# balkce/beamform

Hardware: AMD Instinct MI355X
Metric: stft_frames_per_sec (higher is better)
Workload: dtype f64; 1 GPU; das 8-mic 1024-pt (hop 512), 65536-frame batch per GPU, 1 stream(s), planar input resident in HBM; frames_per_gpu=65536, frames_fed_per_gpu=65536, mics=8, fft=1024, hop=512, streams=1, layout=planar, gather=n/a, parallelism=independent batches x1, input=uniform noise in [-0.5, 0.5), settle_launches_before_warmup=416, forward_transforms_per_frame_pair=6

## Files before the change

beamform_amd/csrc/das_f64_w64.hip:

```cpp
#include <hip/hip_runtime.h>

#include <type_traits>

#include "launch_trace.hpp"
#include "pipeline_kernels.hpp"
#include "w64_f64_dev.hpp"

namespace bf {

namespace {

constexpr int kBlock = 512;
constexpr int kWaves = kBlock / 64;
constexpr int kHop = 512;
constexpr int kTwD = 2 * (1024 + 4 * kTw2RowW64Rot);
constexpr int oTw = 0;
constexpr int oPlane = kTwD;
constexpr int oGain = oPlane + kWaves * kPlaneD;
constexpr int oCross = oGain + 4 * 2048;
constexpr int oFlag = oCross + 512;
constexpr int kWinRow = 18;
constexpr int oWin = oFlag + 8;
constexpr int kLdsD = oWin + 64 * kWinRow;

// ... 180 lines not shown
        BF_STAGE();
        mul_tw<true, 1, 16>(Sr, Si, tw);
        BF_STAGE();
        load_tw1<1, 16>(tw, s_tw1, lane);
        BF_STAGE();
        fft16_core<double, +1, false>(Sr, Si);
        BF_STAGE();
        T1_inv(Sr, Si, row16, wcol);
        BF_STAGE();
        mul_tw<true, 1, 16>(Sr, Si, tw);
        fft16_core<double, +1, false>(Sr, Si);

        float o[16];
#pragma unroll
        for (int j = 0; j < 16; ++j) {
            const float f = (float)Sr[j];
            o[j] = (float)((double)f * wrow[j]);
        }
        const int pw = (w + kWaves - 1) & (kWaves - 1);
        if (t + 1 < T1) {
            float *area = (w < kWaves - 1) ? reinterpret_cast<float *>(plane) : s_cross + (it & 1) * kHop;
            if (w == kWaves - 1 && it >= 2)
                while (s_cons[w] < (int)(t - 2 * kWaves)) __builtin_amdgcn_s_sleep(1);
            asm volatile("" ::: "memory");
#pragma unroll
            for (int j = 0; j < 8; ++j) area[64 * j + lane] = o[j + 8];
            asm volatile("" ::: "memory");
            if (lane == 0) s_ready[w] = (int)t;
        }
        float *yo = ys + t * kHop;
        if (t == T0) {
            if (T0 == 0) {
                const float *ti = a.tail_in + (long)stream * kHop;
#pragma unroll
                for (int j = 0; j < 8; ++j) yo[(unsigned)(64 * j + lane)] = ti[(unsigned)(64 * j + lane)] + o[j];
            } else {
#pragma unroll
                for (int j = 0; j < 8; ++j) atomicAdd(yo + (unsigned)(64 * j + lane), o[j]);
            }
        } else {
            const float *parea = (pw < kWaves - 1) ? reinterpret_cast<const float *>(lds + oPlane + pw * kPlaneD) : s_cross + ((it + 1) & 1) * kHop;
            while (s_ready[pw] < (int)(t - 1)) __builtin_amdgcn_s_sleep(1);
            asm volatile("" ::: "memory");
            float prev[8];
#pragma unroll
            for (int j = 0; j < 8; ++j) prev[j] = parea[64 * j + lane];
            asm volatile("" ::: "memory");
            if (lane == 0) s_cons[pw] = (int)(t - 1);
#pragma unroll
            for (int j = 0; j < 8; ++j) yo[(unsigned)(64 * j + lane)] = prev[j] + o[j];
        }
        if (t == T1 - 1) {
            if (T1 < a.n_frames) {
                float *yn = ys + T1 * kHop;
#pragma unroll
                for (int j = 0; j < 8; ++j) atomicAdd(yn + (unsigned)(64 * j + lane), o[j + 8]);
            } else {
                float *to = a.tail_out + (long)stream * kHop;
#pragma unroll
                for (int j = 0; j < 8; ++j) to[(unsigned)(64 * j + lane)] = o[j + 8];
            }
        }
    }
}


#ifdef BF_PARK_PLAIN
#define BF_PARK_LD(p) (*(const volatile float *)(p))
#else
#define BF_PARK_LD(p) __builtin_nontemporal_load(p)
#endif
constexpr int kGRow = 65;
constexpr int kGMic = 8 * kGRow;
constexpr int kSlots = 64;
constexpr int kTwP = 2 * (960 + 4 * kTw2RowW64Rot);
constexpr int pTw = 0;
constexpr int pPlane = kTwP;
constexpr int pGain = pPlane + kWaves * kPlaneD;
constexpr int pFlag = pGain + 7 * kGMic * 2;
constexpr int kRingR = 32;
constexpr int kRingSlots = kRingR + kWaves;
constexpr int pRing = pFlag + (kSlots + 4) / 2;
constexpr int pWin = pRing + kRingR / 2;
constexpr int kLdsP = pWin + 64 * kWinRow;
static_assert(kLdsP * 8 <= 160 * 1024, "LDS");
static_assert((pGain & 1) == 0 && (pWin & 1) == 0, "16-byte alignment");


typedef volatile __attribute__((address_space(3))) int *lds_int_t;
typedef volatile __attribute__((address_space(3))) unsigned long long *lds_u64_t;
__device__ __forceinline__ int lds_fetch_add(lds_int_t p, int v, int lane) {
    int old = 0;
    if (lane == 0) old = __hip_atomic_fetch_add((__attribute__((address_space(3))) int *)p, v, __ATOMIC_RELAXED, __HIP_MEMORY_SCOPE_WORKGROUP);
    return __builtin_amdgcn_readfirstlane(old);
}
__device__ __forceinline__ unsigned long long lds_fetch_add64(lds_u64_t p, int lane) {
    unsigned long long old = 0;
    if (lane == 0) old = __hip_atomic_fetch_add((__attribute__((address_space(3))) unsigned long long *)p, 1ull, __ATOMIC_RELAXED, __HIP_MEMORY_SCOPE_WORKGROUP);
    const unsigned lo = (unsigned)__builtin_amdgcn_readfirstlane((int)(unsigned)old), hi = (unsigned)__builtin_amdgcn_readfirstlane((int)(unsigned)(old >> 32));
    return ((unsigned long long)hi << 32) | lo;
}
struct DasSched {
    const int4 *chunks;
    unsigned *counter;
    int n_chunks;
};
__device__ __forceinline__ unsigned long long pack_work(unsigned vbase, int chunk, int pairs, int next) {
    return ((unsigned long long)(vbase & 0xFFFFFFu) << 40) | ((unsigned long long)(unsigned)chunk << 20) | ((unsigned long long)(unsigned)pairs << 10) | (unsigned)next;
}
struct PairWork {
    int4 d;
    int pos;
    int len;
    unsigned u;
    bool have;
};
__device__ __forceinline__ int4 load_chunk(const int4 *chunks, int k) {
    const int4 d = chunks[k];
    return int4{__builtin_amdgcn_readfirstlane(d.x), __builtin_amdgcn_readfirstlane(d.y), __builtin_amdgcn_readfirstlane(d.z), k};
}
__device__ __forceinline__ PairWork draw_pair(lds_u64_t work, const DasSched &sc, int lane, const int4 held) {
    PairWork r;
    r.have = false;
    r.d = int4{0, 0, 0, 0};
    r.pos = r.len = 0;
    r.u = 0;
    for (;;) {
        const unsigned long long old = lds_fetch_add64(work, lane);
        const int pos = (int)(old & 1023u), len = (int)((old >> 10) & 1023u), k = (int)((old >> 20) & 0xFFFFFu);
        const unsigned vb = (unsigned)(old >> 40);
        if (k == kChunkEnd) return r;
        if (pos < len) {
            if (k == held.w) r.d = held;
            else r.d = load_chunk(sc.chunks, k);
            r.pos = pos; r.len = len; r.u = vb + (unsigned)pos; r.have = true;
            return r;
        }
        if (pos == len) {
            unsigned k2 = 0;
            if (lane == 0) k2 = __hip_atomic_fetch_add(sc.counter, 1u, __ATOMIC_RELAXED, __HIP_MEMORY_SCOPE_AGENT);
            k2 = (unsigned)__builtin_amdgcn_readfirstlane((int)k2);
            if (k2 >= (unsigned)sc.n_chunks) {
                if (lane == 0) *work = pack_work(vb + (unsigned)len, kChunkEnd, 0, 0);
                return r;
            }
            r.d = load_chunk(sc.chunks, (int)k2);
            r.len = (r.d.z + 1) >> 1;
            r.pos = 0; r.u = vb + (unsigned)len; r.have = true;
            if (lane == 0) *work = pack_work(r.u, (int)k2, r.len, 1);
            return r;
        }
        while ((int)((*work >> 20) & 0xFFFFFu) == k) __builtin_amdgcn_s_sleep(2);
    }
}
__device__ __forceinline__ int claim_boundary(lds_int_t st, unsigned b, int lane) {
    const int base = 4 * (int)(b / kSlots);
    while (st[b & (kSlots - 1)] < base) __builtin_amdgcn_s_sleep(1);
    return lds_fetch_add(st + (b & (kSlots - 1)), 1, lane) - base;
}
__device__ __forceinline__ void publish_boundary(lds_int_t st, unsigned b, int lane) { (void)lds_fetch_add(st + (b & (kSlots - 1)), 2, lane); }
__device__ __forceinline__ void skip_boundary(lds_int_t st, unsigned b, int lane) {
    const int base = 4 * (int)(b / kSlots);
    while (st[b & (kSlots - 1)] < base) __builtin_amdgcn_s_sleep(1);
    (void)lds_fetch_add(st + (b & (kSlots - 1)), 4, lane);
}
__device__ __forceinline__ void await_boundary(lds_int_t st, unsigned b) {
    while (st[b & (kSlots - 1)] - 4 * (int)(b / kSlots) < 3) __builtin_amdgcn_s_sleep(1);
}

#ifdef BF_W64_STATS
__device__ unsigned long long g_stats[256 * 8 * 5];
#define BF_STATS_DECL unsigned long long st_[5] = {0, 0, 0, 0, 0}; const unsigned long long st_t0_ = __builtin_amdgcn_s_memrealtime()
#define BF_STAT(i) (++st_[i])
#define BF_STAT_WAIT_BEGIN const unsigned long long st_w0_ = __builtin_amdgcn_s_memrealtime()
#define BF_STAT_WAIT_END st_[3] += __builtin_amdgcn_s_memrealtime() - st_w0_
#define BF_STATS_FLUSH do { st_[4] = __builtin_amdgcn_s_memrealtime() - st_t0_; if (lane == 0 && blockIdx.x < 256) for (int i_ = 0; i_ < 5; ++i_) g_stats[(blockIdx.x * 8 + w) * 5 + i_] = st_[i_]; } while (0)
#else
#define BF_STATS_DECL
#define BF_STAT(i) ((void)0)
#define BF_STAT_WAIT_BEGIN
#define BF_STAT_WAIT_END
#define BF_STATS_FLUSH
#endif
#ifdef BF_W64_STAMPS
__device__ unsigned long long g_stamps[256 * 8 * 64];
#define BF_STAMP(slot) do { if (lane == 0 && blockIdx.x < 256 && (slot) < 64) g_stamps[(blockIdx.x * 8 + w) * 64 + (slot)] = __builtin_amdgcn_s_memrealtime(); } while (0)
#else
#define BF_STAMP(slot) do { } while (0)
#endif

typedef float il_f4 __attribute__((ext_vector_type(4)));
template <int LG>
__device__ __forceinline__ void il_tile_through_plane(const il_f4 (&v)[4], float *tile, float *dst, int t, int lane) {
    constexpr int M = 1 << LG, R1 = LG == 3 ? 10 : M + 1, spt = 1024 >> LG;
    asm volatile("" : "+v"(lane)::"memory");
#pragma unroll
    for (int i = 0; i < 4; ++i) {
#pragma unroll
        for (int c = 0; c < 4; ++c) {
            const int e = 256 * i + 4 * lane + c;
            tile[(e >> LG) * R1 + (e & (M - 1))] = v[i][c];
        }
    }
    asm volatile("" ::: "memory");
    __builtin_amdgcn_wave_barrier();
#pragma unroll
    for (int j = 0; j < 4; ++j) {
        const int mic = lane & (M - 1), q4 = (lane >> LG) + (64 >> LG) * j;
        il_f4 o;
#pragma unroll
        for (int c = 0; c < 4; ++c) o[c] = tile[(4 * q4 + c) * R1 + mic];
        reinterpret_cast<il_f4 *>(dst + mic * kHop + t * spt)[q4] = o;
    }
    asm volatile("" ::: "memory");
    __builtin_amdgcn_wave_barrier();
}

template <int LAYOUT>
__device__ __forceinline__ void das_f64_pair_body(const DasF64Args &a, const DasSched &sc) {
    __shared__ __attribute__((aligned(16))) double lds[kLdsP];
    const cx<double> *s_tw1 = reinterpret_cast<const cx<double> *>(lds + pTw) - 64;
    const cx<double> *s_tw2 = reinterpret_cast<const cx<double> *>(lds + pTw) + 960;
    const cx<double> *s_gain = reinterpret_cast<const cx<double> *>(lds + pGain);
    lds_int_t s_state = (lds_int_t)(lds + pFlag);
    lds_u64_t s_work = (lds_u64_t)(lds + pFlag + kSlots / 2);
    lds_int_t s_ring = (lds_int_t)(lds + pRing);
    (void)s_ring;

    const int tid = threadIdx.x, lane = tid & 63;
    const int w = __builtin_amdgcn_readfirstlane(tid >> 6);
    const int M = a.n_mics;
    double *plane = lds + pPlane + w * kPlaneD;
    double *wcol = plane + w64_col_rot(lane);
    double *row16 = plane + (lane & 15) * kRS + 16 * (lane >> 4);
    const double *wrow = lds + pWin + lane * kWinRow;
    typedef double cxa __attribute__((ext_vector_type(2)));
    typedef const __attribute__((address_space(3))) cxa *lds_gain_t;
    unsigned gd0 = (unsigned)(size_t)(lds_gain_t)(s_gain + lane);
    asm volatile("" : "+v"(gd0));
    gd0 &= ~15u;
    const unsigned g_mirror = 2u * (unsigned)(size_t)(lds_gain_t)s_gain + 1024u;

    float n0[8], n1[8], n2[8];
#ifndef BF_PAIR_NT
#define BF_PAIR_NT 0
#endif
    auto request = [&](const float *h0, const float *h1, const float *h2) {
#pragma unroll
        for (int j = 0; j < 8; ++j) {
            n0[j] = (BF_PAIR_NT & 2) ? __builtin_nontemporal_load(h0 + (unsigned)(64 * j + lane)) : h0[(unsigned)(64 * j + lane)];
            n1[j] = (BF_PAIR_NT & 1) ? __builtin_nontemporal_load(h1 + (unsigned)(64 * j + lane)) : h1[(unsigned)(64 * j + lane)];
            n2[j] = (BF_PAIR_NT & 4) ? __builtin_nontemporal_load(h2 + (unsigned)(64 * j + lane)) : h2[(unsigned)(64 * j + lane)];
        }
    };
    auto request_pair_mic = [&](int stream, long tA, int m) {
        const float *h1 = a.x + (long)stream * a.stream_stride_x + (long)m * a.mic_stride + tA * kHop;
        const float *h0 = tA >= 1 ? h1 - kHop : a.hist + ((long)stream * M + m) * kHop;
        const float *h2 = tA + 1 < a.n_frames ? h1 + kHop : h1;
        request(h0, h1, h2);
    };
    float q0[8], q1[8], q2[8];
    const double inv_m = 1.0 / (double)M;
    float e0[8], e1[8], e2[8];
    const int NT = a.n_tr, XM = a.extra_mic;
    auto request_extra = [&](bool on, int stream, long tA) {
        if (!on) {
#pragma unroll
            for (int j = 0; j < 8; ++j) e0[j] = e1[j] = e2[j] = 0.f;
            return;
        }
        const float *h1 = a.x + (long)stream * a.stream_stride_x + (long)XM * a.mic_stride + tA * kHop;
        const float *h0 = tA >= 1 ? h1 - kHop : a.hist + ((long)stream * M + XM) * kHop;
        const float *h2 = tA + 1 < a.n_frames ? h1 + kHop : h1;
#pragma unroll
        for (int j = 0; j < 8; ++j) {
            e0[j] = h0[(unsigned)(64 * j + lane)];
            e1[j] = h1[(unsigned)(64 * j + lane)];
            e2[j] = h2[(unsigned)(64 * j + lane)];
        }
    };

    struct RingHops { const float *h, *a, *b; };
    typedef float f4 __attribute__((ext_vector_type(4)));
    const int lgM = 31 - __builtin_clz((unsigned)M);
    float *ringb = LAYOUT == 1 ? a.ring + (size_t)blockIdx.x * kRingSlots * M * kHop : nullptr;
    auto ring_slot = [&](unsigned j) { return ringb + (size_t)(j & (kRingR - 1)) * M * kHop; };
    auto il_load2 = [&](const float *src, int unit, f4 (&v)[2][4]) {
        const f4 *s4 = reinterpret_cast<const f4 *>(src);
#pragma unroll
        for (int tt = 0; tt < 2; ++tt) {
            const int t = 2 * unit + tt;
            if (2 * t < M) {
#pragma unroll
                for (int i = 0; i < 4; ++i) v[tt][i] = s4[t * 256 + i * 64 + lane];
            } else {
#pragma unroll
                for (int i = 0; i < 4; ++i) v[tt][i] = f4{0.f, 0.f, 0.f, 0.f};
            }
        }
    };
    auto il_store2 = [&](const f4 (&v)[2][4], float *dst, int unit) {
        float *tile = reinterpret_cast<float *>(plane);
#pragma unroll
        for (int tt = 0; tt < 2; ++tt) {
            const int t = 2 * unit + tt;
            if (2 * t < M) {
                if (lgM == 3) il_tile_through_plane<3>(v[tt], tile, dst, t, lane);
                else if (lgM == 2) il_tile_through_plane<2>(v[tt], tile, dst, t, lane);
                else il_tile_through_plane<1>(v[tt], tile, dst, t, lane);
            }
// ... 1 lines not shown
    };
    auto prepare_pair = [&](const PairWork &pw) {
        RingHops r;
        const unsigned u2 = 2u * pw.u;
        const int sA = (int)(u2 & (kRingR - 1)), gen4 = 4 * (int)(u2 / kRingR);
        float *dA = ring_slot(u2), *dB = ring_slot(u2 + 1), *dH = ringb + (size_t)(kRingR + w) * M * kHop;
        const long tA = pw.d.y + 2L * pw.pos;
        const float *xs = a.x + (long)pw.d.x * a.stream_stride_x;
        while (s_ring[sA] < gen4 || s_ring[sA + 1] < gen4) __builtin_amdgcn_s_sleep(1);
        f4 v0[2][4], v1[2][4];
        const bool two = tA + 1 < a.n_frames, first = pw.pos == 0, wide = M > 4;
        const float *srcA = xs + tA * (long)kHop * M, *srcB = srcA + (long)kHop * M;
        const float *srcH = tA >= 1 ? srcA - (long)kHop * M : a.hist + (long)pw.d.x * M * kHop;
        il_load2(srcA, 0, v0);
        if (wide) il_load2(srcA, 1, v1);
        il_store2(v0, dA, 0);
        if (two) il_load2(srcB, 0, v0);
        if (wide) il_store2(v1, dA, 1);
        if (two && wide) il_load2(srcB, 1, v1);
        if (two) il_store2(v0, dB, 0);
        if (first) il_load2(srcH, 0, v0);
        if (two && wide) il_store2(v1, dB, 1);
        if (first && wide) il_load2(srcH, 1, v1);
        if (first) il_store2(v0, dH, 0);
        if (first && wide) il_store2(v1, dH, 1);
        __builtin_amdgcn_fence(__ATOMIC_RELEASE, "workgroup");
        (void)lds_fetch_add(s_ring + sA, 2, lane);
        (void)lds_fetch_add(s_ring + sA + 1, 2, lane);
        r.a = dA;
        r.b = two ? dB : dA;
        r.h = dH;
        if (!first) {
            const unsigned jp = u2 - 1;
            const int sP = (int)(jp & (kRingR - 1)), genp = 4 * (int)(jp / kRingR);
            while (s_ring[sP] - genp < 2) __builtin_amdgcn_s_sleep(1);
            r.h = ring_slot(jp);
        }
        __builtin_amdgcn_fence(__ATOMIC_ACQUIRE, "workgroup");
        return r;
    };
    auto release_pair = [&](const PairWork &pw, bool has_t) {
        const unsigned u2 = 2u * pw.u;
        (void)lds_fetch_add(s_ring + (u2 & (kRingR - 1)), 2, lane);
        (void)lds_fetch_add(s_ring + ((u2 + 1) & (kRingR - 1)), has_t ? 1 : 2, lane);
        if (pw.pos > 0) (void)lds_fetch_add(s_ring + ((u2 - 1) & (kRingR - 1)), 1, lane);
    };
    auto request_ring_mic = [&](const RingHops &r, int m) { request(r.h + m * kHop, r.a + m * kHop, r.b + m * kHop); };
    auto request_ring_extra = [&](bool on, const RingHops &r) {
        if (!on) {
#pragma unroll
            for (int j = 0; j < 8; ++j) e0[j] = e1[j] = e2[j] = 0.f;
            return;
        }
#pragma unroll
        for (int j = 0; j < 8; ++j) {
            e0[j] = r.h[XM * kHop + (unsigned)(64 * j + lane)];
            e1[j] = r.a[XM * kHop + (unsigned)(64 * j + lane)];
            e2[j] = r.b[XM * kHop + (unsigned)(64 * j + lane)];
        }
    };
    RingHops curR{nullptr, nullptr, nullptr};
    (void)curR;

    BF_STAMP(0);
#ifdef BF_W64_STAMPS
    if (lane == 0 && blockIdx.x < 256) g_stamps[(blockIdx.x * 8 + w) * 64 + 59] = __builtin_amdgcn_s_memtime();
#endif
    PairWork cur;
    cur.d = load_chunk(sc.chunks, (int)blockIdx.x);
    cur.len = (cur.d.z + 1) >> 1;
    const int n_static = cur.len < kWaves ? cur.len : kWaves;
    cur.pos = w;
    cur.u = (unsigned)w;
    cur.have = w < n_static;
    if (LAYOUT == 0 && cur.have) {
        request_pair_mic(cur.d.x, cur.d.y + 2L * w, a.slot_mic[0]);
        request_extra(XM >= 0, cur.d.x, cur.d.y + 2L * w);
    } else {
        request_extra(false, 0, 0);
    }
    {
        const f64x2 *tw2 = a.tw + 64;
        f64x2 *ltw = reinterpret_cast<f64x2 *>(lds + pTw), *lg = reinterpret_cast<f64x2 *>(lds + pGain);
#pragma unroll 4
        for (int i = tid; i < kTwP / 2; i += kBlock) ltw[i] = tw2[i];
        for (int k = 0; k < NT; ++k) {
            const f64x2 *g2 = a.gains_mic + a.slot_mic[k] * kGMic;
#pragma unroll 2
            for (int i = tid; i < kGMic; i += kBlock) lg[k * kGMic + i] = g2[i];
        }
#pragma unroll 2
        for (int i = tid; i < 1024; i += kBlock) lds[pWin + (i & 63) * kWinRow + (i >> 6)] = a.win[i];
        if (tid < kSlots) s_state[tid] = 0;
        if (tid < kRingR) s_ring[tid] = 0;
        if (tid == 0) *s_work = pack_work(0u, (int)blockIdx.x, cur.len, n_static);
    }
    __syncthreads();
    BF_STAMP(1);
    BF_STATS_DECL;
    int it = 0;
    if (!cur.have) {
        cur = draw_pair(s_work, sc, lane, cur.d);
        if (LAYOUT == 0 && cur.have) {
            request_pair_mic(cur.d.x, cur.d.y + 2L * cur.pos, a.slot_mic[0]);
            request_extra(XM >= 0, cur.d.x, cur.d.y + 2L * cur.pos);
        }
    }
    while (cur.have) {
        if constexpr (LAYOUT == 1) {
            curR = prepare_pair(cur);
            request_ring_mic(curR, a.slot_mic[0]);
            request_ring_extra(XM >= 0, curR);
        }
        const int stream = cur.d.x;
        const long T0 = cur.d.y, T1 = T0 + cur.d.z;
        const long tA = T0 + 2L * cur.pos;
        const bool pair = tA + 1 < T1;
        const long tL = pair ? tA + 1 : tA;
        const unsigned u = cur.u;
        const bool has_t = cur.pos + 1 < cur.len, has_h = cur.pos > 0;
        float *ys = a.y + (long)stream * a.n_frames * kHop;
        PairWork nxt;
        nxt.have = false;
        const float *hp0 = a.x + (long)stream * a.stream_stride_x + tA * kHop;
        const float *hist0 = a.hist + (long)stream * M * kHop;
        const bool first_hop = tA < 1, last_hop = !(tA + 1 < a.n_frames);
        (void)hp0; (void)hist0; (void)first_hop; (void)last_hop;

        double Sr[16], Si[16];
        auto one_mic = [&](const int k, auto first_tag) {
            constexpr bool FIRST = decltype(first_tag)::value;
            double re[16], im[16];
#ifndef BF_PAIR_NO_VMWAIT
            if constexpr (!FIRST) __builtin_amdgcn_s_waitcnt(0x0F70);
#endif
            if (FIRST && XM >= 0) {
#pragma unroll
                for (int j = 0; j < 8; ++j) {
                    const double w0 = wrow[j], w1 = wrow[j + 8];
                    const double c = (double)n1[j] + (double)e1[j];
                    const double t = ((double)n0[j] + (double)e0[j]) * w0;
                    re[j] = fma(c, w1, t);
                    re[j + 8] = fma(-c, w1, t);
                    const double t2 = c * w0, u2 = (double)n2[j] + (double)e2[j];
                    im[j] = fma(u2, w1, t2);
                    im[j + 8] = fma(-u2, w1, t2);
                }
            } else {
#pragma unroll
                for (int j = 0; j < 8; ++j) {
                    const double w0 = wrow[j], w1 = wrow[j + 8];
                    const double c = (double)n1[j];
                    const double t = (double)n0[j] * w0;
                    re[j] = fma(c, w1, t);
                    re[j + 8] = fma(-c, w1, t);
                    const double t2 = c * w0, u2 = (double)n2[j];
                    im[j] = fma(u2, w1, t2);
                    im[j + 8] = fma(-u2, w1, t2);
                }
            }
            if (__builtin_expect(!pair, 0)) {
#ifndef BF_PAIR_CNDMASK
                asm volatile("" ::: "memory");
#endif
#pragma unroll
                for (int j = 0; j < 16; ++j) im[j] = 0.0;
            }
            if (k + 1 < NT) {
                if constexpr (LAYOUT == 1) request_ring_mic(curR, a.slot_mic[k + 1]);
                else request_pair_mic(stream, tA, a.slot_mic[k + 1]);
            } else {
                nxt = draw_pair(s_work, sc, lane, cur.d);
                if constexpr (LAYOUT == 0) {
                    if (nxt.have) request_pair_mic(nxt.d.x, nxt.d.y + 2L * nxt.pos, a.slot_mic[0]);
                    else request_pair_mic(stream, tA, a.slot_mic[0]);
                }
// ... 27 lines not shown
            const lds_gain_t gm = (lds_gain_t)(size_t)((g_mirror + (unsigned)(2 * k * kGMic * 16)) - (gd0 + (unsigned)(k * kGMic * 16)));
            BF_STAGE();
#pragma unroll
            for (int r = 0; r < 8; ++r)
                g[r] = (r & 3) < 2 ? gd[(2 * (r >> 2) + (r & 3)) * kGRow] : gm[(2 * (3 - (r >> 2)) + 3 - (r & 3)) * kGRow];
            BF_STAGE();
            w64_fwd_p3<double>(re, im);
            BF_STAGE();
#pragma unroll
            for (int r = 8; r < 16; ++r)
                g[r] = (r & 3) < 2 ? gd[(2 * (r >> 2) + (r & 3)) * kGRow] : gm[(2 * (3 - (r >> 2)) + 3 - (r & 3)) * kGRow];
            BF_STAGE();
#pragma unroll
            for (int r = 0; r < 16; ++r) {
                if (r == 8) BF_STAGE();
                const double gx = g[r].x, gy = (r & 3) < 2 ? g[r].y : -g[r].y;
                if constexpr (FIRST) {
                    Sr[r] = fma(-gy, im[r], gx * re[r]);
                    Si[r] = fma(gy, re[r], gx * im[r]);
                } else {
                    Sr[r] = fma(-gy, im[r], fma(gx, re[r], Sr[r]));
                    Si[r] = fma(gy, re[r], fma(gx, im[r], Si[r]));
                }
            }
        };
        one_mic(0, std::true_type{});
        for (int k = 1; k < NT; ++k) one_mic(k, std::false_type{});
        float *yo = ys + tA * kHop;
        cx<double> tw[15];
        BF_STAGE();
        {
            const float *h0 = LAYOUT == 1 ? curR.h : (first_hop ? hist0 : hp0 - kHop), *h1 = LAYOUT == 1 ? curR.a : hp0;
            const float *h2 = LAYOUT == 1 ? curR.b : (last_hop ? hp0 : hp0 + kHop);
#pragma unroll
            for (int j = 0; j < 8; ++j) {
                q0[j] = h0[(unsigned)(64 * j + lane)];
                q1[j] = h1[(unsigned)(64 * j + lane)];
                q2[j] = h2[(unsigned)(64 * j + lane)];
            }
            if constexpr (LAYOUT == 0) request_extra(XM >= 0 && nxt.have, nxt.d.x, nxt.d.y + 2L * nxt.pos);
        }
        BF_STAGE();
        load_tw2<1, 16>(tw, s_tw2, lane);
        BF_STAGE();
        w64_inv_p3<double>(Sr, Si);
        w64_T2_any<false>(Sr, Si, row16 - 16 * (lane >> 4), lane >> 4);
        BF_STAGE();
        mul_tw<true, 1, 16>(Sr, Si, tw);
        BF_STAGE();
        load_tw1<1, 16>(tw, s_tw1, lane);
        BF_STAGE();
        fft16_core<double, +1, false>(Sr, Si);
        BF_STAGE();
        T1_inv(Sr, Si, row16, wcol);
        BF_STAGE();
        mul_tw<true, 1, 16>(Sr, Si, tw);
        fft16_core<double, +1, false>(Sr, Si);

#pragma unroll
        for (int j = 0; j < 8; ++j) {
            const double w0 = wrow[j], w1 = wrow[j + 8];
            const double c = (double)q1[j];
            Sr[j] = fma((double)q0[j] * w0, inv_m, Sr[j]);
            Sr[j + 8] = fma(c * w1, inv_m, Sr[j + 8]);
            Si[j] = fma(c * w0, inv_m, Si[j]);
            Si[j + 8] = fma((double)q2[j] * w1, inv_m, Si[j + 8]);
        }
        float oA[16], tl[8];
        if (pair) {
#pragma unroll
            for (int j = 0; j < 8; ++j) {
                const float f1 = (float)Si[j + 8];
                tl[j] = (float)((double)f1 * wrow[j + 8]);
            }
        } else {
#pragma unroll
            for (int j = 0; j < 8; ++j) {
                const float f1 = (float)Sr[j + 8];
                tl[j] = (float)((double)f1 * wrow[j + 8]);
            }
        }
        float *yn = ys + (tL + 1) * kHop;
        int oT = -1, oH = -1;
        if (has_t) {
            oT = claim_boundary(s_state, u, lane);
            if (oT == 0) {
#pragma unroll
                for (int j = 0; j < 8; ++j) yn[(unsigned)(64 * j + lane)] = tl[j];
            }
        } else {
            skip_boundary(s_state, u, lane);
        }
#pragma unroll
        for (int j = 0; j < 16; ++j) {
            const float f = (float)Sr[j];
            oA[j] = (float)((double)f * wrow[j]);
        }
        if (pair) {
            float *y1 = ys + (tA + 1) * kHop;
#pragma unroll
            for (int j = 0; j < 8; ++j) {
                const float f0 = (float)Si[j];
                const float b0 = (float)((double)f0 * wrow[j]);
                y1[(unsigned)(64 * j + lane)] = oA[j + 8] + b0;
            }
        }
        if (has_h) {
            oH = claim_boundary(s_state, u - 1, lane);
            if (oH == 0) {
#pragma unroll
                for (int j = 0; j < 8; ++j) yo[(unsigned)(64 * j + lane)] = oA[j];
            }
        } else if (T0 == 0) {
            const float *ti = a.tail_in + (long)stream * kHop;
#pragma unroll
            for (int j = 0; j < 8; ++j) yo[(unsigned)(64 * j + lane)] = ti[(unsigned)(64 * j + lane)] + oA[j];
        } else {
#pragma unroll
            for (int j = 0; j < 8; ++j) atomicAdd(yo + (unsigned)(64 * j + lane), oA[j]);
        }
        if (oT == 0 || oH == 0) {
            __builtin_amdgcn_fence(__ATOMIC_RELEASE, "workgroup");
            if (oT == 0) publish_boundary(s_state, u, lane);
            if (oH == 0) publish_boundary(s_state, u - 1, lane);
        }
        if (oT > 0) {
            BF_STAT(2);
            BF_STAT_WAIT_BEGIN;
            await_boundary(s_state, u);
            BF_STAT_WAIT_END;
            __builtin_amdgcn_fence(__ATOMIC_ACQUIRE, "workgroup");
            float o[8];
#pragma unroll
            for (int j = 0; j < 8; ++j) o[j] = BF_PARK_LD(yn + (unsigned)(64 * j + lane));
#pragma unroll
            for (int j = 0; j < 8; ++j) yn[(unsigned)(64 * j + lane)] = tl[j] + o[j];
        } else {
            BF_STAT(0);
        }
        if (oH > 0) {
            BF_STAT(2);
            BF_STAT_WAIT_BEGIN;
            await_boundary(s_state, u - 1);
            BF_STAT_WAIT_END;
            __builtin_amdgcn_fence(__ATOMIC_ACQUIRE, "workgroup");
            float o[8];
#pragma unroll
            for (int j = 0; j < 8; ++j) o[j] = BF_PARK_LD(yo + (unsigned)(64 * j + lane));
#pragma unroll
            for (int j = 0; j < 8; ++j) yo[(unsigned)(64 * j + lane)] = o[j] + oA[j];
        } else {
            BF_STAT(1);
        }
        if (!has_t) {
            if (T1 < a.n_frames) {
                float *ynx = ys + T1 * kHop;
#pragma unroll
                for (int j = 0; j < 8; ++j) atomicAdd(ynx + (unsigned)(64 * j + lane), tl[j]);
            } else {
                float *to = a.tail_out + (long)stream * kHop;
#pragma unroll
                for (int j = 0; j < 8; ++j) to[(unsigned)(64 * j + lane)] = tl[j];
                if (a.hist_out != nullptr) {
                    float *ho = a.hist_out + (long)stream * M * kHop;
                    const float *xs = a.x + (long)stream * a.stream_stride_x;
                    for (int m = 0; m < M; ++m) {
                        const float *xl = xs + (long)m * a.mic_stride + tL * kHop;
#pragma unroll
                        for (int j = 0; j < 8; ++j) ho[m * kHop + 64 * j + lane] = xl[(unsigned)(64 * j + lane)];
                    }
                }
            }
        }
        if constexpr (LAYOUT == 1) {
            asm volatile("" ::: "memory");
            release_pair(cur, has_t);
        }
        cur = nxt;
        ++it;
    }
    BF_STATS_FLUSH;
#ifdef BF_W64_STAMPS
    if (lane == 0 && blockIdx.x < 256) {
        g_stamps[(blockIdx.x * 8 + w) * 64 + 63] = __builtin_amdgcn_s_memrealtime();
        g_stamps[(blockIdx.x * 8 + w) * 64 + 60] = __builtin_amdgcn_s_memtime();
        g_stamps[(blockIdx.x * 8 + w) * 64 + 62] = (unsigned long long)it;
        g_stamps[(blockIdx.x * 8 + w) * 64 + 61] = (unsigned long long)__builtin_amdgcn_s_getreg(((4 - 1) << 11) | (0 << 6) | 20);
    }
#endif
    (void)it;
}

__global__ __launch_bounds__(kBlock) void das_f64_pair_kernel(DasF64Args a, DasSched sc) { das_f64_pair_body<0>(a, sc); }
__global__ __launch_bounds__(kBlock) void das_f64_ring_kernel(DasF64Args a, DasSched sc) { das_f64_pair_body<1>(a, sc); }

constexpr int kSchedPerBlock = 8;
__global__ __launch_bounds__(32 * kSchedPerBlock) void das_f64_sched_kernel(DasSchedPlan p, int4 *chunks, unsigned *counter, float *y, long n_frames, int n_streams) {
    const int k = blockIdx.x * kSchedPerBlock + (int)(threadIdx.x >> 5), l = (int)(threadIdx.x & 31);
    if (k >= p.n_chunks) return;
    int stream;
    long t0, n;
    das_f64_chunk(p, n_frames, n_streams, k, &stream, &t0, &n);
    if (l == 0) {
        chunks[k] = int4{stream, (int)t0, (int)n, 0};
        if (k == 0) *counter = (unsigned)p.grid;
    }
    if (t0 > 0) {
        float4 *h = reinterpret_cast<float4 *>(y + ((long)stream * n_frames + t0) * kHop);
        for (int i = l; i < kHop / 4; i += 32) h[i] = float4{0.f, 0.f, 0.f, 0.f};
    }
}

__global__ __launch_bounds__(256) void interleaved_to_planar_kernel(const float *x, float *out, long tiles_per_stream, int M, long in_stream_stride,
                                                                    long out_mic_stride, long out_stream_stride) {
    __shared__ float s_t[256 * 9];
    const int tid = threadIdx.x;
    const long s = blockIdx.x / tiles_per_stream, tile = blockIdx.x - s * tiles_per_stream;
    const float4 *src = reinterpret_cast<const float4 *>(x + s * in_stream_stride + tile * 256 * M);
    const int R = M + 1;
    for (int i = tid; i < 64 * M; i += 256) {
        const float4 v = src[i];
        const int e = 4 * i;
        s_t[(e / M) * R + e % M] = v.x;
        s_t[((e + 1) / M) * R + (e + 1) % M] = v.y;
        s_t[((e + 2) / M) * R + (e + 2) % M] = v.z;
        s_t[((e + 3) / M) * R + (e + 3) % M] = v.w;
    }
    __syncthreads();
    float *dst = out + s * out_stream_stride + tile * 256;
    for (int j = tid; j < 64 * M; j += 256) {
        const int m = j >> 6, q = j & 63;
// ... 63 lines not shown
```

beamform_amd/csrc/pipeline.hip:

```cpp
#include "pipeline.hpp"

#include <hip/hip_runtime.h>

#include <cmath>
#include <utility>
#include <vector>

#include "device_mem.hpp"
#include "fft1024.hpp"
#include "pipeline_kernels.hpp"
#include "switches.hpp"

namespace bf {

namespace {

class BinPipelineImpl : public Engine {
    static constexpr int kMaxCols = BF_MAX_INTERF + 1;
   public:
    BinPipelineImpl(const bf_config &c, int n_cus) : cfg_(c), n_cus_(n_cus) {
        M_ = c.n_mics;
        H_ = c.hop;
        N_ = 2 * c.hop;
        NQ_ = problems_per_frame(N_);
// ... 179 lines not shown
    size_t nlms_bytes() const {
        return time_node_ ? (size_t)S_ * (2 * (M_ - 1) + 1) * cfg_.gsc_filter_size * sizeof(float) : 0;
    }

    int copy_state(char *p, bool to_host) {
        ENGINE_HIP(hipDeviceSynchronize());
        struct Seg { void *d; size_t n; } segs[] = {
            {d_hist2_[hist_cur_].get(), hist_elems() * sizeof(float)}, {d_tail_[tail_cur_].get(), tail_elems() * sizeof(float)},
            {d_zhist_.get(), zhist_bytes()}, {d_gssW_.get(), gss_bytes()}, {d_mpf_.get(), mpf_bytes()}, {d_smooth_.get(), smooth_bytes()},
            {d_nlms_.get(), nlms_bytes()}};
        for (auto &s : segs) {
            if (!s.n) continue;
            if (to_host)
                ENGINE_HIP(hipMemcpy(p, s.d, s.n, hipMemcpyDeviceToHost));
            else
                ENGINE_HIP(hipMemcpy(s.d, p, s.n, hipMemcpyHostToDevice));
            p += s.n;
        }
        return BF_OK;
    }

    bf_config cfg_;
    int n_cus_, M_, MF_, NP_, S_, D_, So_, R_, KP1_, Phist_;
    const bool cov_node_ = cfg_.algo == BF_MVDR || cfg_.algo == BF_LCMV;
    const bool band_node_ = cov_node_ || cfg_.algo == BF_GSS;
    const bool time_node_ = cfg_.algo == BF_GSC;
    const bool single_ch_ = cfg_.algo == BF_MCRA;
    const bool post_amp_ = band_node_;
    const bool yraw_target_ = cfg_.algo == BF_PHASEMPF || time_node_;
    int skip_lo_, skip_hi_ = 0;
    int band_yh_lo_ = 0, band_yh_hi_;
    bool z48_ = false;
    size_t zsz_ = sizeof(f64x2);
    int H_ = 512, N_ = 1024, NQ_ = 514, YS_ = 516;
    const KernelSet *ks_ = nullptr;
    long steer_dir_stride_ = 0;
    std::vector<double> freqs_;
    DeviceBuffer<f64x2> d_tw_;
    DeviceBuffer<f32x2> d_tw32_;
    DeviceBuffer<double> d_win_, d_freq_;
    DeviceBuffer<f64x2> d_steer_[2];
    struct DasTables { DeviceBuffer<f64x2> gains_w64, gains_mic; DasSlots slots; } das_[2];
    DeviceBuffer<f64x2> d_tw_w64_;
    DeviceBuffer<char> d_das_sched_;
    int steer_cur_ = 0;
    DeviceBuffer<f64x2> d_track_;
    DeviceBuffer<f64x2> d_track_retired_;
    int track_n_ = 0;
    DeviceBuffer<float> d_hist2_[2];
    int hist_cur_ = 0;
    DeviceBuffer<float> d_tail_[2];
    int tail_cur_ = 0;
    DeviceBuffer<char> d_zhist_;
    DeviceBuffer<f64x2> d_gssW_;
    DeviceBuffer<double> d_mpf_;
    DeviceBuffer<double> d_smooth_;
    DeviceBuffer<float> d_nlms_;
    unsigned long long gss_reset_mask_ = ~0ull;
    DeviceBuffer<char> d_Z_;
    DeviceBuffer<char> d_Yh_;
    DeviceBuffer<float> d_yraw_;
    DeviceBuffer<float> d_planar_;
    DeviceBuffer<float> d_frames_;
};

int BinPipelineImpl::run_das_one_launch(const float *x, long F, float *y, hipStream_t stream, int layout, long mic_stride, const RunSnapshot &snap) {
    const Switches &sw = switches();
    if (!das_one_launch_shape() || sw.fused_bins != 1 || snap.das.gains_w64 == nullptr) return kDeclined;
    const DasSlots &sl = snap.das.slots;
    const DasF64Launch d = das_f64_decide(DasF64Shape{layout, M_, S_, n_cus_, F, sl.mic0_unit, snap.das.gains_mic && d_das_sched_.get(), sl.n_tr,
                                                      sw.das_il_ring, sw.das_f64_sched});
    if (d.path == DasF64Path::kChain) return kDeclined;
    ENGINE_HIP(d_planar_.reserve((d.scratch_bytes + sizeof(float) - 1) / sizeof(float)));
    float *const hist = d_hist2_[hist_cur_].get();
    DasF64Args da;
    da.x = x; da.hist = hist; da.hist_out = d_hist2_[hist_cur_ ^ 1].get(); da.y = y;
    da.tail_in = d_tail_[tail_cur_].get(); da.tail_out = d_tail_[tail_cur_ ^ 1].get();
    da.win = d_win_.get(); da.n_frames = F; da.mic_stride = mic_stride;
    da.stream_stride_x = (long)M_ * F * H_; da.n_streams = S_; da.n_mics = M_; da.run_len = 1; da.layout = layout;
    da.gains = snap.das.gains_w64; da.gains_mic = snap.das.gains_mic; da.tw = d_tw_w64_.get();
    da.mic0_unit = sl.mic0_unit ? 1 : 0; da.n_tr = sl.n_tr; da.extra_mic = sl.extra_mic;
    for (int k = 0; k < 8; ++k) da.slot_mic[k] = sl.slot_mic[k];
    da.sched_ws = d_das_sched_.get(); da.sched_ws_bytes = d_das_sched_.get() ? das_f64_sched_ws_bytes() : 0;
    ENGINE_HIP(enqueue_das_f64(da, d, d_planar_.get(), stream, kev0, kev1, &kev_recorded));
    if (d.writes_hist)
        hist_cur_ ^= 1;
    else
        ENGINE_HIP(carry_last_hop(hist, x, F, H_, M_, S_, layout, mic_stride, (long)F * H_ * M_, stream));
    tail_cur_ ^= 1;
    return BF_OK;
}

int BinPipelineImpl::run(const float *x, long F, float *y, f64x2 *spectrum, hipStream_t stream, int layout, long mic_stride,
                         const RunSnapshot &snap) {
    const int rc = (spectrum || snap.track) ? kDeclined : run_das_one_launch(x, F, y, stream, layout, mic_stride, snap);
    return rc == kDeclined ? run_chain(x, F, y, spectrum, stream, layout, mic_stride, snap) : rc;
}

int BinPipelineImpl::run_chain(const float *x, long F, float *y, f64x2 *spectrum, hipStream_t stream, int layout, long mic_stride,
                               const RunSnapshot &snap) {
    const Switches &sw = switches();
    const ChainPlan p = chain_decide(ChainShape{cfg_.algo, N_, layout, M_, S_, cfg_.n_dirs > 1 ? cfg_.n_dirs : 1, snap.kp1, cfg_.past_windows,
                                                cfg_.precision, spectrum != nullptr, F, n_cus_, cfg_.gsc_filter_size, cfg_.smooth_size,
                                                band_yh_lo_, band_yh_hi_, (reinterpret_cast<size_t>(y) & 15) == 0, sw.fused_bins,
                                                sw.stft_small, sw.stft_split, sw.mvdr_group, sw.gss_group, sw.gsc_serial, R_, snap.track != nullptr});
    float *const hist = d_hist2_[hist_cur_].get();
    const long FT = Phist_ + F;
    ENGINE_HIP(d_Z_.reserve(p.z_bytes));
    ENGINE_HIP(d_Yh_.reserve(p.yh_bytes));
    ENGINE_HIP(d_yraw_.reserve(p.yraw_elems));
    ENGINE_HIP(d_frames_.reserve(p.frames_elems));
    f64x2 *const Z = (f64x2 *)d_Z_.get();
    f64x2 *const Yh = (f64x2 *)d_Yh_.get();
    const size_t frame_elems = (size_t)NP_ * N_;

    if (Phist_ > 0)
        ENGINE_HIP(hipMemcpy2DAsync(Z, (size_t)FT * frame_elems * zsz_, d_zhist_.get(), (size_t)Phist_ * frame_elems * zsz_,
                                  (size_t)Phist_ * frame_elems * zsz_, (size_t)S_, hipMemcpyDeviceToDevice, stream));

    StftArgs sa;
    sa.x = x; sa.hist = hist; sa.Z = Z; sa.tw = d_tw_.get(); sa.win = d_win_.get();
    sa.n_frames = F; sa.frames_ws = FT; sa.frame_off = Phist_; sa.mic_stride = mic_stride;
    sa.stream_stride_x = (long)M_ * F * H_; sa.n_streams = S_; sa.n_mics = M_; sa.n_fft_mics = MF_; sa.layout = layout;
    sa.skip_lo = skip_lo_; sa.skip_hi = skip_hi_;
    sa.z48 = p.z48 ? 1 : 0; sa.run_len = 1; sa.tw_w64 = d_tw_w64_.get();
    sa.halve = cov_node_ ? 1 : 0;
    if (time_node_ && spectrum) {
        ENGINE_HIP(hipMemsetAsync(spectrum, 0, (size_t)S_ * F * N_ * sizeof(f64x2), stream));
        spectrum = nullptr;
    }
    BinsArgs ba;
    ba.Z = Z; ba.Yh = Yh; ba.spectrum = spectrum; ba.steer = snap.steer; ba.freqs = d_freq_.get();
    ba.n_frames = F; ba.frames_ws = FT; ba.frame_off = Phist_; ba.n_streams = So_; ba.n_mics = MF_; ba.kp1 = snap.kp1;
    ba.n_dirs = D_; ba.steer_dir_stride = snap.steer_dir_stride;
    ba.z48 = p.z48 ? 1 : 0;
    ba.cfg = cfg_; ba.gssW = d_gssW_.get(); ba.mpf = d_mpf_.get(); ba.gss_reset_mask = snap.gss_reset_mask;
    ba.yh32 = p.yh32 ? 1 : 0; ba.mpf32 = p.mpf32 ? 1 : 0; ba.yh_lo = p.yh_lo; ba.yh_hi = p.yh_hi;
    ba.gss_rows = p.rows;
    if (p.track) {
        ba.track = snap.track; ba.track_tables = snap.track_tables; ba.track_n = snap.track_n; ba.track_stride = (long)M_ * N_;
    }
    if (p.rec_istft()) {
        ba.rec_istft = 1;
        ba.rec_y = d_yraw_.get(); ba.rec_tail_in = d_tail_[tail_cur_].get(); ba.rec_tail_out = d_tail_[tail_cur_ ^ 1].get();
        ba.rec_tw_w64 = d_tw_w64_.get(); ba.rec_win = d_win_.get();
    }
    IstftArgs ia;
    ia.Yh = Yh; ia.y = yraw_target_ ? d_yraw_.get() : y; ia.tail_in = d_tail_[tail_cur_].get();
    ia.tail_out = d_tail_[tail_cur_ ^ 1].get(); ia.tw = d_tw_.get(); ia.win = d_win_.get(); ia.n_frames = F;
    ia.n_streams = So_ * p.rows;
    ia.tw32 = d_tw32_.get();
    ia.tw_w64 = d_tw_w64_.get();
    ia.yh32 = ba.yh32; ia.yh_lo = ba.yh_lo; ia.yh_hi = ba.yh_hi;
    if (p.mpf32) {
        ia.Yh = Yh + (size_t)So_ * F * YS_;
        ia.yh32 = 1; ia.yh_lo = 0; ia.yh_hi = NQ_ - 1;
    }
    ia.frames = d_frames_.get();
    ia.post_amp = post_amp_ ? cfg_.out_amp : 1.0;
    ia.use_post_amp = post_amp_ ? 1 : 0;

    if (p.fused())
        ENGINE_HIP(ks_->stft_bins(p, sa, ba, n_cus_, stream));
    else
        ENGINE_HIP(ks_->stft(p, sa, n_cus_, stream));
    ENGINE_HIP(carry_last_hop(hist, x, F, H_, M_, S_, layout, mic_stride, (long)F * H_ * M_, stream));
// ... 23 lines not shown
```

beamform_amd/csrc/pipeline_kernels.hpp:

```cpp
#pragma once

#include <hip/hip_runtime.h>

#include <cstdint>

#include "../../include/bfcore.h"
#include "chain_plan.hpp"
#include "das_f64_plan.hpp"
#include "geometry.hpp"

namespace bf {

#ifdef BF_NFFT
#define BF_CAT2_(a, b) a##b
#define BF_CAT2(a, b) BF_CAT2_(a, b)
#define BF_NTAG BF_CAT2(n, BF_NFFT)
#endif

constexpr int problems_per_frame(int nfft) { return nfft / 2 + 2; }
constexpr int yh_stride(int nfft) { return nfft / 2 + 4; }
constexpr int kMpfVecs = 7;
#ifdef BF_NFFT
namespace BF_NTAG {
constexpr int kN = BF_NFFT;
// ... 12 lines not shown
    const float *x;
    const float *hist;
    f64x2 *Z;
    const f64x2 *tw;
    const double *win;
    long n_frames, frames_ws, frame_off, mic_stride, stream_stride_x;
    int n_streams, n_mics, layout;
    int n_fft_mics;
    int skip_lo, skip_hi;
    int z48;
    int halve = 0;
    int run_len;
    const f64x2 *tw_w64 = nullptr;
};

struct BinsArgs {
    const f64x2 *Z;
    f64x2 *Yh;
    int yh32;
    int yh_lo, yh_hi;
    f64x2 *spectrum;
    const f64x2 *steer;
    const double *freqs;
    long n_frames, frames_ws, frame_off;
    int n_streams, n_mics, kp1;
    int n_dirs;
    long steer_dir_stride;
    bf_config cfg;
    f64x2 *gssW;
    double *mpf;
    unsigned long long gss_reset_mask;
    int z48;
    int rec_istft = 0;
    float *rec_y = nullptr;
    const float *rec_tail_in = nullptr;
    float *rec_tail_out = nullptr;
    const f64x2 *rec_tw_w64 = nullptr;
    const double *rec_win = nullptr;
    int mpf32;
    int gss_rows = 1;
    const int32_t *track = nullptr;
    const f64x2 *track_tables = nullptr;
    int track_n = 0;
    long track_stride = 0;
};
struct IstftArgs {
    const f64x2 *Yh;
    int yh32;
    int yh_lo, yh_hi;
    float *y;
    const float *tail_in;
    float *tail_out;
    const f64x2 *tw;
    const f32x2 *tw32;
    const f64x2 *tw_w64 = nullptr;
    float *frames;
    const double *win;
    long n_frames;
    int n_streams;
    double post_amp;
    int use_post_amp;
};
struct DasF64Args {
    const float *x;
    const float *hist;
    float *y;
    const float *tail_in;
    float *tail_out;
    const f64x2 *gains;
    const f64x2 *tw;
    const double *win;
    long n_frames, mic_stride, stream_stride_x;
    int n_streams, n_mics, run_len;
    int layout = 0;
    float *hist_out = nullptr;
    const f64x2 *gains_mic = nullptr;
    int n_tr = 0, extra_mic = -1;
    int slot_mic[8] = {1, 2, 3, 4, 5, 6, 7, 0};
    int mic0_unit = 0;
    void *sched_ws = nullptr;
    size_t sched_ws_bytes = 0;
    float *ring = nullptr;
    size_t ring_bytes = 0;
};

hipError_t enqueue_das_f64(DasF64Args a, const DasF64Launch &d, float *scratch, hipStream_t s, hipEvent_t kev0, hipEvent_t kev1, bool *kev_recorded);

#ifdef BF_NFFT
namespace BF_NTAG {
hipError_t launch_stft(const ChainPlan &p, const StftArgs &a, int n_cus, hipStream_t s);
hipError_t launch_bins(const ChainPlan &p, const BinsArgs &a, int n_cus, hipStream_t s);
hipError_t launch_stft_bins_fused(const ChainPlan &p, const StftArgs &a, const BinsArgs &b, int n_cus, hipStream_t s);
hipError_t launch_pointwise(const ChainPlan &p, const BinsArgs &a, hipStream_t s);
hipError_t launch_mpf_mask(const ChainPlan &p, const BinsArgs &a, hipStream_t s);
hipError_t launch_mcra_node(const BinsArgs &a, hipStream_t s);
hipError_t launch_mvdr_lcmv(const ChainPlan &p, const BinsArgs &a, int n_cus, hipStream_t s);
hipError_t launch_gss(const ChainPlan &p, const BinsArgs &a, hipStream_t s);
hipError_t launch_gsc_align(const BinsArgs &a, hipStream_t s);
hipError_t launch_bins_end(const ChainPlan &p, const BinsArgs &a, hipStream_t s);
hipError_t launch_expand_spectrum(const f64x2 *Yh, f64x2 *spectrum, long frames, hipStream_t s);
hipError_t launch_istft(const ChainPlan &p, const IstftArgs &a, int n_cus, hipStream_t s);
hipError_t launch_gsc_nlms(const ChainPlan &p, const float *aligned, float *y, float *state, long n_samples, int n_streams, int n_mics,
                           const bf_config &cfg, hipStream_t s);
hipError_t launch_smooth(const ChainPlan &p, const float *yraw, float *y, double *state, long n_frames, int n_streams, hipStream_t s);
}
#endif

struct KernelSet {
    int nfft;
    hipError_t (*stft)(const ChainPlan &, const StftArgs &, int, hipStream_t);
    hipError_t (*bins)(const ChainPlan &, const BinsArgs &, int, hipStream_t);
    hipError_t (*stft_bins)(const ChainPlan &, const StftArgs &, const BinsArgs &, int, hipStream_t);
    hipError_t (*istft)(const ChainPlan &, const IstftArgs &, int, hipStream_t);
    hipError_t (*smooth)(const ChainPlan &, const float *, float *, double *, long, int, hipStream_t);
    hipError_t (*gsc_nlms)(const ChainPlan &, const float *, float *, float *, long, int, int, const bf_config &, hipStream_t);
};
const KernelSet *kernel_set_n128();
const KernelSet *kernel_set_n256();
const KernelSet *kernel_set_n512();
const KernelSet *kernel_set_n1024();
const KernelSet *kernel_set_n2048();
const KernelSet *kernel_set_n4096();
const KernelSet *kernel_set_n8192();
inline const KernelSet *kernel_set(int nfft) {
    switch (nfft) {
        case 128: return kernel_set_n128();
        case 256: return kernel_set_n256();
        case 512: return kernel_set_n512();
        case 1024: return kernel_set_n1024();
        case 2048: return kernel_set_n2048();
        case 4096: return kernel_set_n4096();
        case 8192: return kernel_set_n8192();
        default: return nullptr;
    }
}

}
```

beamform_amd/csrc/switches.hpp:

```cpp
#pragma once

#include <cstdlib>
#include <string>

namespace bf {

struct Switches {
    static int num(const char *name, int unset) { const char *v = getenv(name); return v ? atoi(v) : unset; }
    static const char *keep(const char *v) { static std::string s; return v ? (s = v).c_str() : nullptr; }
    const char *const das_f64_sched = keep(getenv("BF_DAS_F64_SCHED"));
    const int das_interleave = num("BF_DAS_INTERLEAVE", 1);
    const int das_il_ring = num("BF_DAS_IL_RING", 1);
    const int das_split2048 = num("BF_DAS_SPLIT2048", 3);
    const int das_shared_dirs = num("BF_DAS_SHARED_DIRS", 6);
    const int fused_bins = num("BF_FUSED_BINS", 1);
    const bool stft_small = num("BF_STFT_SMALL", 1) != 0;
    const bool stft_split = num("BF_STFT_SPLIT", 1) != 0;
    const bool mvdr_group = num("BF_MVDR_GROUP", 0) != 0;
    const int mvdr_tile = num("BF_MVDR_TILE", 0);
    const int gss_group = num("BF_GSS_GROUP", -1);
    const bool gsc_serial = num("BF_GSC_SERIAL", 0) == 1;
};

inline const Switches &switches() {
    static const Switches sw;
    return sw;
}

}
```

Baseline: 138.5 million frames/s.

## Park overlap-add boundary halves in LDS slots instead of global memory

Adds a small pool of LDS park slots with compare-exchange ownership words. The first wave to reach a hop boundary parks its half-frame there, and the second wave reads it back from LDS, avoiding a global write, an acquire fence and a nontemporal reload. When all slots are busy it falls back to the old global path. The prologue table fill is also rewritten as one batched load-then-store pass so the global loads can overlap, and the LDS footprint grows slightly, which may reduce occupancy.

```diff
diff --git a/beamform_amd/csrc/das_f64_w64.hip b/beamform_amd/csrc/das_f64_w64.hip
--- a/beamform_amd/csrc/das_f64_w64.hip
+++ b/beamform_amd/csrc/das_f64_w64.hip
@@ -286,9 +286,13 @@
 constexpr int kRingSlots = kRingR + kWaves;
 constexpr int pRing = pFlag + (kSlots + 4) / 2;
 constexpr int pWin = pRing + kRingR / 2;
-constexpr int kLdsP = pWin + 64 * kWinRow;
+constexpr int kPark = 6;
+constexpr int pPark = pWin + 64 * kWinRow;
+constexpr int pOwner = pPark + kPark * (kHop / 2);
+constexpr int kLdsP = pOwner + 4;
 static_assert(kLdsP * 8 <= 160 * 1024, "LDS");
-static_assert((pGain & 1) == 0 && (pWin & 1) == 0, "16-byte alignment");
+static_assert((pGain & 1) == 0 && (pWin & 1) == 0 && (pPark & 1) == 0, "16-byte alignment");
+static_assert(kPark <= 8, "owner words");
 
 
 typedef volatile __attribute__((address_space(3))) int *lds_int_t;
@@ -371,6 +375,24 @@
 __device__ __forceinline__ void await_boundary(lds_int_t st, unsigned b) {
     while (st[b & (kSlots - 1)] - 4 * (int)(b / kSlots) < 3) __builtin_amdgcn_s_sleep(1);
 }
+__device__ __forceinline__ unsigned park_slot(unsigned b, unsigned n) { return n == (unsigned)kPark ? b % (unsigned)kPark : b % n; }
+__device__ __forceinline__ bool park_take(lds_int_t owner, unsigned b, unsigned n, int lane) {
+    if (n == 0) return false;
+    int got = 1;
+    if (lane == 0) {
+        int expected = 0;
+        __hip_atomic_compare_exchange_strong((__attribute__((address_space(3))) int *)(owner + park_slot(b, n)), &expected, (int)(b + 1u), __ATOMIC_RELAXED, __ATOMIC_RELAXED,
+                                             __HIP_MEMORY_SCOPE_WORKGROUP);
+        got = expected;
+    }
+    return __builtin_amdgcn_readfirstlane(got) == 0;
+}
+__device__ __forceinline__ bool park_holds(lds_int_t owner, unsigned b, unsigned n) { return n != 0 && owner[park_slot(b, n)] == (int)(b + 1u); }
+__device__ __forceinline__ void park_free(lds_int_t owner, unsigned b, unsigned n, int lane) {
+    asm volatile("s_waitcnt lgkmcnt(0)" ::: "memory");
+    if (lane == 0) owner[park_slot(b, n)] = 0;
+}
+#define BF_LGKM_DONE() asm volatile("s_waitcnt lgkmcnt(0)" ::: "memory")
 
 #ifdef BF_W64_STATS
 __device__ unsigned long long g_stats[256 * 8 * 5];
@@ -422,7 +444,7 @@
 
 template <int LAYOUT>
 __device__ __forceinline__ void das_f64_pair_body(const DasF64Args &a, const DasSched &sc) {
-    __shared__ __attribute__((aligned(16))) double lds[kLdsP];
+    __shared__ __attribute__((aligned(16))) double lds[LAYOUT == 1 ? pPark : kLdsP];
     const cx<double> *s_tw1 = reinterpret_cast<const cx<double> *>(lds + pTw) - 64;
     const cx<double> *s_tw2 = reinterpret_cast<const cx<double> *>(lds + pTw) + 960;
     const cx<double> *s_gain = reinterpret_cast<const cx<double> *>(lds + pGain);
@@ -430,6 +452,9 @@
     lds_u64_t s_work = (lds_u64_t)(lds + pFlag + kSlots / 2);
     lds_int_t s_ring = (lds_int_t)(lds + pRing);
     (void)s_ring;
+    float *s_park = reinterpret_cast<float *>(lds + pPark);
+    lds_int_t s_owner = (lds_int_t)(lds + pOwner);
+    const unsigned n_park = LAYOUT == 1 ? 0u : (unsigned)__builtin_amdgcn_readfirstlane(a.park_lds < 0 || a.park_lds > kPark ? kPark : a.park_lds);
 
     const int tid = threadIdx.x, lane = tid & 63;
     const int w = __builtin_amdgcn_readfirstlane(tid >> 6);
@@ -597,6 +622,7 @@
     {
         const f64x2 *tw2 = a.tw + 64;
         f64x2 *ltw = reinterpret_cast<f64x2 *>(lds + pTw), *lg = reinterpret_cast<f64x2 *>(lds + pGain);
+#ifdef BF_PAIR_TABLE_LOOPS
 #pragma unroll 4
         for (int i = tid; i < kTwP / 2; i += kBlock) ltw[i] = tw2[i];
         for (int k = 0; k < NT; ++k) {
@@ -606,7 +632,35 @@
         }
 #pragma unroll 2
         for (int i = tid; i < 1024; i += kBlock) lds[pWin + (i & 63) * kWinRow + (i >> 6)] = a.win[i];
+#else
+        constexpr int kTwE = kTwP / 2, kFill = (kTwE + 7 * kGMic + kBlock - 1) / kBlock;
+        const int n_fill = kTwE + NT * kGMic;
+        typedef double d2 __attribute__((ext_vector_type(2)));
+        d2 v[kFill];
+#pragma unroll
+        for (int r = 0; r < kFill; ++r) {
+            int e = tid + r * kBlock;
+            e = e < n_fill ? e : n_fill - 1;
+            const int ge = e - kTwE, k = ge / kGMic;
+            int mic = a.slot_mic[0];
+#pragma unroll
+            for (int kk = 1; kk < 7; ++kk) mic = k == kk ? a.slot_mic[kk] : mic;
+            const size_t st = (size_t)(tw2 + e), sg = (size_t)(a.gains_mic + ((long)(mic - k) * kGMic + ge));
+            v[r] = *reinterpret_cast<const d2 *>(e < kTwE ? st : sg);
+        }
+        const double wv0 = a.win[tid], wv1 = a.win[tid + kBlock];
+        asm volatile("" ::: "memory");
+#pragma unroll
+        for (int r = 0; r < kFill; ++r) {
+            const int e = tid + r * kBlock;
+            d2 *dst = reinterpret_cast<d2 *>(e < kTwE ? ltw + e : lg + (e - kTwE));
+            if (e < n_fill) *dst = v[r];
+        }
+        lds[pWin + (tid & 63) * kWinRow + (tid >> 6)] = wv0;
+        lds[pWin + (tid & 63) * kWinRow + ((tid + kBlock) >> 6)] = wv1;
+#endif
         if (tid < kSlots) s_state[tid] = 0;
+        if (LAYOUT == 0 && tid < 8) s_owner[tid] = 0;
         if (tid < kRingR) s_ring[tid] = 0;
         if (tid == 0) *s_work = pack_work(0u, (int)blockIdx.x, cur.len, n_static);
     }
@@ -800,11 +854,21 @@
         }
         float *yn = ys + (tL + 1) * kHop;
         int oT = -1, oH = -1;
+        bool gT = false, gH = false;
         if (has_t) {
             oT = claim_boundary(s_state, u, lane);
             if (oT == 0) {
-#pragma unroll
-                for (int j = 0; j < 8; ++j) yn[(unsigned)(64 * j + lane)] = tl[j];
+                if (park_take(s_owner, u, n_park, lane)) {
+                    float *ps = s_park + park_slot(u, n_park) * kHop;
+#pragma unroll
+                    for (int j = 0; j < 8; ++j) ps[64 * j + lane] = tl[j];
+                    BF_LGKM_DONE();
+                    publish_boundary(s_state, u, lane);
+                } else {
+                    gT = true;
+#pragma unroll
+                    for (int j = 0; j < 8; ++j) yn[(unsigned)(64 * j + lane)] = tl[j];
+                }
             }
         } else {
             skip_boundary(s_state, u, lane);
@@ -826,8 +890,17 @@
         if (has_h) {
             oH = claim_boundary(s_state, u - 1, lane);
             if (oH == 0) {
-#pragma unroll
-                for (int j = 0; j < 8; ++j) yo[(unsigned)(64 * j + lane)] = oA[j];
+                if (park_take(s_owner, u - 1, n_park, lane)) {
+                    float *ps = s_park + park_slot(u - 1, n_park) * kHop;
+#pragma unroll
+                    for (int j = 0; j < 8; ++j) ps[64 * j + lane] = oA[j];
+                    BF_LGKM_DONE();
+                    publish_boundary(s_state, u - 1, lane);
+                } else {
+                    gH = true;
+#pragma unroll
+                    for (int j = 0; j < 8; ++j) yo[(unsigned)(64 * j + lane)] = oA[j];
+                }
             }
         } else if (T0 == 0) {
             const float *ti = a.tail_in + (long)stream * kHop;
@@ -837,20 +910,28 @@
 #pragma unroll
             for (int j = 0; j < 8; ++j) atomicAdd(yo + (unsigned)(64 * j + lane), oA[j]);
         }
-        if (oT == 0 || oH == 0) {
+        if (gT || gH) {
             __builtin_amdgcn_fence(__ATOMIC_RELEASE, "workgroup");
-            if (oT == 0) publish_boundary(s_state, u, lane);
-            if (oH == 0) publish_boundary(s_state, u - 1, lane);
+            if (gT) publish_boundary(s_state, u, lane);
+            if (gH) publish_boundary(s_state, u - 1, lane);
         }
         if (oT > 0) {
             BF_STAT(2);
             BF_STAT_WAIT_BEGIN;
             await_boundary(s_state, u);
             BF_STAT_WAIT_END;
-            __builtin_amdgcn_fence(__ATOMIC_ACQUIRE, "workgroup");
+            asm volatile("" ::: "memory");
             float o[8];
-#pragma unroll
-            for (int j = 0; j < 8; ++j) o[j] = BF_PARK_LD(yn + (unsigned)(64 * j + lane));
+            if (park_holds(s_owner, u, n_park)) {
+                const float *ps = s_park + park_slot(u, n_park) * kHop;
+#pragma unroll
+                for (int j = 0; j < 8; ++j) o[j] = ps[64 * j + lane];
+                park_free(s_owner, u, n_park, lane);
+            } else {
+                __builtin_amdgcn_fence(__ATOMIC_ACQUIRE, "workgroup");
+#pragma unroll
+                for (int j = 0; j < 8; ++j) o[j] = BF_PARK_LD(yn + (unsigned)(64 * j + lane));
+            }
 #pragma unroll
             for (int j = 0; j < 8; ++j) yn[(unsigned)(64 * j + lane)] = tl[j] + o[j];
         } else {
@@ -861,10 +942,18 @@
             BF_STAT_WAIT_BEGIN;
             await_boundary(s_state, u - 1);
             BF_STAT_WAIT_END;
-            __builtin_amdgcn_fence(__ATOMIC_ACQUIRE, "workgroup");
+            asm volatile("" ::: "memory");
             float o[8];
-#pragma unroll
-            for (int j = 0; j < 8; ++j) o[j] = BF_PARK_LD(yo + (unsigned)(64 * j + lane));
+            if (park_holds(s_owner, u - 1, n_park)) {
+                const float *ps = s_park + park_slot(u - 1, n_park) * kHop;
+#pragma unroll
+                for (int j = 0; j < 8; ++j) o[j] = ps[64 * j + lane];
+                park_free(s_owner, u - 1, n_park, lane);
+            } else {
+                __builtin_amdgcn_fence(__ATOMIC_ACQUIRE, "workgroup");
+#pragma unroll
+                for (int j = 0; j < 8; ++j) o[j] = BF_PARK_LD(yo + (unsigned)(64 * j + lane));
+            }
 #pragma unroll
             for (int j = 0; j < 8; ++j) yo[(unsigned)(64 * j + lane)] = o[j] + oA[j];
         } else {
diff --git a/beamform_amd/csrc/pipeline.hip b/beamform_amd/csrc/pipeline.hip
--- a/beamform_amd/csrc/pipeline.hip
+++ b/beamform_amd/csrc/pipeline.hip
@@ -285,6 +285,7 @@
     da.mic0_unit = sl.mic0_unit ? 1 : 0; da.n_tr = sl.n_tr; da.extra_mic = sl.extra_mic;
     for (int k = 0; k < 8; ++k) da.slot_mic[k] = sl.slot_mic[k];
     da.sched_ws = d_das_sched_.get(); da.sched_ws_bytes = d_das_sched_.get() ? das_f64_sched_ws_bytes() : 0;
+    da.park_lds = sw.das_park_lds;
     ENGINE_HIP(enqueue_das_f64(da, d, d_planar_.get(), stream, kev0, kev1, &kev_recorded));
     if (d.writes_hist)
         hist_cur_ ^= 1;
diff --git a/beamform_amd/csrc/pipeline_kernels.hpp b/beamform_amd/csrc/pipeline_kernels.hpp
--- a/beamform_amd/csrc/pipeline_kernels.hpp
+++ b/beamform_amd/csrc/pipeline_kernels.hpp
@@ -118,6 +118,7 @@
     size_t sched_ws_bytes = 0;
     float *ring = nullptr;
     size_t ring_bytes = 0;
+    int park_lds = -1;
 };
 
 hipError_t enqueue_das_f64(DasF64Args a, const DasF64Launch &d, float *scratch, hipStream_t s, hipEvent_t kev0, hipEvent_t kev1, bool *kev_recorded);
diff --git a/beamform_amd/csrc/switches.hpp b/beamform_amd/csrc/switches.hpp
--- a/beamform_amd/csrc/switches.hpp
+++ b/beamform_amd/csrc/switches.hpp
@@ -11,6 +11,7 @@
     const char *const das_f64_sched = keep(getenv("BF_DAS_F64_SCHED"));
     const int das_interleave = num("BF_DAS_INTERLEAVE", 1);
     const int das_il_ring = num("BF_DAS_IL_RING", 1);
+    const int das_park_lds = num("BF_DAS_PARK_LDS", -1);
     const int das_split2048 = num("BF_DAS_SPLIT2048", 3);
     const int das_shared_dirs = num("BF_DAS_SHARED_DIRS", 6);
     const int fused_bins = num("BF_FUSED_BINS", 1);
```

Result: no change. 139.8 million frames/s, median of 6 (+0.9%).
